# SchlomoFeng/GDN

Measured on AMD Instinct MI355X. Metric: sliding-windows/sec forward+anomaly-score, SWaT-shape (127 sensors, W=15), higher is better.
Workload: dtype f32; 1 GPU; BASELINE configs[2]: SWaT-shape eval forward + anomaly score; sensors=127, window=15, topk=30, dim=64, out_layer_num=1, batch=512, batches_per_launch=64, windows_per_launch=32768, storage=fp32, multi_gpu_measured=False, hip_graph=True, forward_streams=3, parallelism=single GPU

## Files before the change

gdn_amd/csrc/gdn_forward_dense.hip:

```cpp
#include "gdn_common.hpp"

#include <stdlib.h>

int gdn_dense_fused_op_d128(int op, const void* args, int bf16, unsigned* plan_out, long long* bytes,
                            hipStream_t st);

namespace {

typedef _Float16 h8 __attribute__((ext_vector_type(8)));
typedef _Float16 h2 __attribute__((ext_vector_type(2)));
typedef __bf16 b8 __attribute__((ext_vector_type(8)));
typedef __bf16 b2 __attribute__((ext_vector_type(2)));
typedef float f32x16 __attribute__((ext_vector_type(16)));
typedef unsigned int u32x4 __attribute__((ext_vector_type(4)));

enum { FMT_F16 = 0, FMT_BF16 = 1 };
#define GDN_LOG2E 1.44269504088896340736f
#define GDN_F16_ALPHA_SCALE 4096.0f
#define GDN_F16_X_SCALE 8.0f
#define GDN_F16_XT_SCALE 8.0f
#define GDN_F16_Z_SCALE 8.0f

template <int FMT>
struct Fmt;
// ... 48 lines not shown
    for (int j = 0; j < 4; ++j) {
      const unsigned p = Fmt<FMT>::pk(r[2 * j], r[2 * j + 1]);
      out[t][j] = p;
      if (t + 1 < NTERM) {
        r[2 * j] = Fmt<FMT>::res0(p, r[2 * j]);
        r[2 * j + 1] = Fmt<FMT>::res1(p, r[2 * j + 1]);
      }
    }
}

__host__ __device__ __forceinline__ int pos_of_source(int src) {
  return (src & ~12) | ((src & 4) << 1) | ((src & 8) >> 1);
}

enum { DMODE_FUSED = 0 };

template <int NT, int DC, int WK, int SL, int FMT>
struct DCfg {
  static constexpr int KS = 2 * NT;
  static constexpr int ROWS = 32 * NT;
  static constexpr int THREADS = 64 * NT;
  static constexpr int AROW = KS * 32 + 16;
  static constexpr int AWAVE = 32 * AROW;
  static constexpr bool XAGG = FMT == FMT_F16;
  static constexpr int MCB = XAGG ? 1 : DC;
  static constexpr int NPX = FMT == FMT_F16 ? 2 : 1;
  static constexpr int NTL = FMT == FMT_F16 ? 2 : 3;
  static constexpr int NTXIN = FMT == FMT_F16 ? 2 : 1;
  static constexpr int XP = 16 * WK + 4;
  static constexpr int XU = 8 * WK;
  static constexpr bool XHALF = XAGG && WK == 1;
  static constexpr int XFL = XHALF ? 16 : 32;
  static constexpr int XFRAG = 2 * XFL * 16;
  static constexpr int OFF_A = 0;
  static constexpr int OFF_XF = NT * AWAVE;
  static constexpr int OFF_XS = OFF_XF + KS * MCB * NPX * XFRAG;
  static constexpr int OFF_SI = OFF_XS + (XAGG ? 0 : ROWS * XP * 4);
  static constexpr int OFF_SJ = OFF_SI + ROWS * 4;
  static constexpr int OFF_EC = OFF_SJ + ROWS * 4;
  static constexpr int OFF_CS = OFF_EC + 4 * 32 * DC * 4;
  static constexpr int CS_WORDS = XAGG ? 0 : 3 * ROWS;
  static constexpr int LDS = OFF_CS + CS_WORDS * 4;
  static constexpr int CW = 16 * WK, RS = THREADS / CW;
  static __host__ __device__ constexpr int xrow0(int xsl) { return XAGG ? 16 * (xsl >> 1) + 4 * (xsl & 1) : xsl; }
  static __host__ __device__ constexpr int xro(int u) {
    return XAGG ? 16 * NT * (u >> 3) + 8 * ((u & 7) >> 2) + (u & 3) : u * RS;
  }
  static constexpr int LDS_UNIT = 1280;
  static constexpr int LDS_ALLOC = (LDS + LDS_UNIT - 1) / LDS_UNIT * LDS_UNIT;
  static constexpr int WGS = !(DC == 2 && NT >= 3 && SL <= 16 && WK == 1) ? 1
                             : XAGG && 3 * LDS_ALLOC <= 160 * 1024 ? 3 : 2;
};

struct DArgs {
  const void* x;
  int series_len;
  int series_first;
  int batch, n, w, pitch, d;
  const float* lin_w;
  const float* node_terms;
  const uint16_t* nbr;
  const float* gnn_bias;
  const float* emb;
  const float* bn1;
  const float* bn2;
  const float* out_w;
  const float* out_b;
  float* out;
  const unsigned* plan;
  const float* key_gt;
  double* keys;
  int key_pitch;
  int* range_flag;
};

__device__ __forceinline__ float lds_f32(const char* smem, int byte_off) {
  return *reinterpret_cast<const float*>(smem + byte_off);
}
__device__ __forceinline__ u32x4 lds_frag(const char* smem, int byte_off) {
  return *reinterpret_cast<const u32x4*>(smem + byte_off);
}

template <int SL, int FMT, bool WANT_ALPHA>
__device__ __forceinline__ void softmax_split(const char* smem, int si_off, const int (&sjoff)[SL],
                                              unsigned (&ph)[SL / 2], unsigned (&pl)[SL / 2], float (&alpha)[SL]) {
  using F = Fmt<FMT>;
  const float sti = lds_f32(smem, si_off);
  float e[SL];
#pragma unroll
  for (int q = 0; q < SL; ++q) e[q] = lds_f32(smem, sjoff[q]);
  __builtin_amdgcn_sched_barrier(0);
  float m = -3.0e38f;
#pragma unroll
  for (int q = 0; q < SL; ++q) {
    e[q] = leaky(sti + e[q]);
    m = fmaxf(m, e[q]);
  }
  m = fmaxf(m, dpp_f<GDN_DPP_XOR1>(m));
  float sum = 0.f;
#pragma unroll
  for (int q = 0; q < SL; ++q) {
    e[q] = __builtin_amdgcn_exp2f(e[q] - m);
    sum += e[q];
  }
  sum += dpp_f<GDN_DPP_XOR1>(sum);
  constexpr float ASC = FMT == FMT_F16 ? GDN_F16_ALPHA_SCALE : 1.f;
  const float inv = __builtin_amdgcn_rcpf(fmaf(sum, 1.f / ASC, GDN_SOFTMAX_EPS / ASC));
#pragma unroll
  for (int q = 0; q < SL; q += 2) {
    const float a0 = e[q] * inv, a1 = e[q + 1] * inv;
    ph[q / 2] = F::pk(a0, a1);
    pl[q / 2] = F::pk(F::res0(ph[q / 2], a0), F::res1(ph[q / 2], a1));
    if constexpr (WANT_ALPHA) {
      alpha[q] = a0 * (1.f / ASC);
      alpha[q + 1] = a1 * (1.f / ASC);
    }
  }
}

template <int SL>
__device__ __forceinline__ void scatter_terms(char* smem, const int (&scoff)[SL], const unsigned (&p)[SL / 2]) {
#pragma unroll
  for (int q = 0; q < SL; q += 2) {
    *reinterpret_cast<uint16_t*>(smem + scoff[q]) = (uint16_t)p[q / 2];
    *reinterpret_cast<uint16_t*>(smem + scoff[q + 1]) = (uint16_t)(p[q / 2] >> 16);
  }
}

template <int M, int CTRL, int N>
__device__ __forceinline__ void halve_sources(float (&r)[N], bool upper) {
  static_assert(2 * M <= N, "");
#pragma unroll
  for (int i = 0; i < M; ++i) {
    const float keep = upper ? r[i + M] : r[i], give = upper ? r[i] : r[i + M];
    r[i] = keep + dpp_f<CTRL>(give);
  }
}

#ifdef GDN_STAMPS
__device__ unsigned long long g_dense_stamps[64];
#define GDN_STAMP(i)                                                                      \
  if (blockIdx.x == 0 && threadIdx.x == 0) {                                              \
    unsigned long long t_;                                                                \
    asm volatile("s_memrealtime %0\n\ts_waitcnt lgkmcnt(0)" : "=s"(t_)::"memory");       \
    g_dense_stamps[i] = t_;                                                               \
  }
#else
#define GDN_STAMP(i)
#endif

__device__ __forceinline__ float ld_or(const float* p, int idx, bool ok, float other = 0.f) {
  const float v = p[ok ? idx : 0];
  return ok ? v : other;
}

template <int NT, int DC, int WK, int SL, int FMT>
struct LaneConsts {
  using C = DCfg<NT, DC, WK, SL, FMT>;
  int sjoff[SL], scoff[SL];
  u32x4 bl[DC][WK][C::NTL], bs[WK][C::NTL];
  float sk, sp, sadd;
  float e2[DC][16];
  float out_b;
  static constexpr int WORDS = 2 * SL + 4 * DC * WK * C::NTL + (C::XAGG ? 3 : 4 * WK * C::NTL) + 16 * DC + 1;
  static constexpr int TABLE_WORDS = 4 * 32 * DC + C::CS_WORDS;
  static constexpr size_t LIMIT_WORD = (size_t)TABLE_WORDS + (size_t)WORDS * C::THREADS;
  static constexpr size_t PLAN_BYTES = (LIMIT_WORD + 1) * 4;

  template <class Fn>
  __device__ __forceinline__ void each_word(Fn&& f) {
    int i = 0;
#pragma unroll
    for (int q = 0; q < SL; ++q) f(i++, reinterpret_cast<unsigned&>(sjoff[q]));
#pragma unroll
    for (int q = 0; q < SL; ++q) f(i++, reinterpret_cast<unsigned&>(scoff[q]));
#pragma unroll
    for (int cb = 0; cb < DC; ++cb)
#pragma unroll
      for (int wk = 0; wk < WK; ++wk)
#pragma unroll
        for (int t = 0; t < C::NTL; ++t)
#pragma unroll
          for (int e = 0; e < 4; ++e) {
            unsigned tmp = bl[cb][wk][t][e];
            f(i++, tmp);
            bl[cb][wk][t][e] = tmp;
          }
    if constexpr (C::XAGG) {
      f(i++, reinterpret_cast<unsigned&>(sk));
      f(i++, reinterpret_cast<unsigned&>(sp));
      f(i++, reinterpret_cast<unsigned&>(sadd));
    } else {
#pragma unroll
      for (int wk = 0; wk < WK; ++wk)
#pragma unroll
        for (int t = 0; t < C::NTL; ++t)
#pragma unroll
          for (int e = 0; e < 4; ++e) {
            unsigned tmp = bs[wk][t][e];
            f(i++, tmp);
            bs[wk][t][e] = tmp;
          }
    }
#pragma unroll
    for (int cb = 0; cb < DC; ++cb)
#pragma unroll
      for (int r = 0; r < 16; ++r) f(i++, reinterpret_cast<unsigned&>(e2[cb][r]));
    f(i++, reinterpret_cast<unsigned&>(out_b));
  }
};

template <int NT, int DC, int WK, int SL, int FMT>
__device__ __forceinline__ void compute_lane_consts(const DArgs& a, LaneConsts<NT, DC, WK, SL, FMT>& k) {
  using C = DCfg<NT, DC, WK, SL, FMT>;
  constexpr bool FOLD = FMT == FMT_F16;
  const int tid = threadIdx.x, lane = tid & 63, wv = tid >> 6;
  const int l32 = lane & 31, h = lane >> 5;
  const int n = a.n, w = a.w, d = 32 * DC;
  const int ti = 32 * wv + (lane >> 1);
  const int half = lane & 1;
  {
    const uint16_t* row = a.nbr + (size_t)min(ti, n - 1) * a.pitch + half * SL;
#pragma unroll
    for (int q = 0; q < SL; ++q) {
      const int jj = (int)row[q];
      const int j = ti < n ? jj : n;
      k.sjoff[q] = C::OFF_SJ + j * 4;
      k.scoff[q] = C::OFF_A + wv * C::AWAVE + (lane >> 1) * C::AROW + pos_of_source(j) * 2;
    }
  }
#pragma unroll
  for (int cb = 0; cb < DC; ++cb) {
    const int c = cb * 32 + l32;
    const float sc = FOLD ? a.bn1[c] * GDN_F16_X_SCALE : 1.f;
#pragma unroll
    for (int wk = 0; wk < WK; ++wk) {
      float v[8];
#pragma unroll
      for (int j = 0; j < 8; ++j) {
        const int kk = wk * 16 + (C::XAGG ? 8 * (j >> 2) + 4 * h + (j & 3) : 8 * h + j);
        v[j] = ld_or(a.lin_w, c * w + kk, kk < w) * sc;
      }
      split8<FMT, C::NTL>(v, k.bl[cb][wk]);
    }
  }
  if constexpr (C::XAGG) {
    const int xcol = tid & (C::CW - 1), kind = xcol / (C::CW / 2);
    const int pcol = WK == 1 ? xcol ^ 15 : xcol ^ 16;
    const int row = C::xrow0(tid / C::CW) + C::xro(xcol & (C::CW / 2 - 1));
    k.sk = ld_or(a.node_terms, kind * GDN_A_PITCH + xcol, xcol < w) * GDN_LOG2E;
    k.sp = ld_or(a.node_terms, kind * GDN_A_PITCH + pcol, pcol < w) * GDN_LOG2E;
    k.sadd = ld_or(a.node_terms, 2 * GDN_A_PITCH + kind * n + row, row < n) * GDN_LOG2E;
    if (kind == 1 && row == n) k.sadd = -INFINITY;
  } else {
#pragma unroll
    for (int wk = 0; wk < WK; ++wk) {
      float v[8];
#pragma unroll
      for (int j = 0; j < 8; ++j) {
        const int kk = wk * 16 + 8 * h + j;
        v[j] = ld_or(a.node_terms, l32 * GDN_A_PITCH + kk, l32 < 2) * GDN_LOG2E;
      }
      split8<FMT, C::NTL>(v, k.bs[wk]);
    }
  }
  const int tgt = 32 * wv + l32;
#pragma unroll
  for (int cb = 0; cb < DC; ++cb)
#pragma unroll
    for (int r = 0; r < 16; ++r) {
      const int c = cb * 32 + (r & 3) + 8 * (r >> 2) + 4 * h;
      k.e2[cb][r] = ld_or(a.emb, tgt * d + c, tgt < n) * a.bn2[c] *
                    (FMT == FMT_F16 ? 1.f / (GDN_F16_Z_SCALE * GDN_F16_X_SCALE) : 1.f);
    }
  k.out_b = a.out_b[0];
}

template <int NT, int DC, int FMT>
__device__ __forceinline__ void compute_tables(const DArgs& a, float* dst) {
  constexpr int ROWS = 32 * NT, THREADS = 64 * NT, d = 32 * DC;
  const int tid = threadIdx.x, n = a.n;
  for (int c = tid; c < d; c += THREADS) {
    dst[c] = a.bn2[d + c];
    dst[d + c] = a.out_w[c];
    dst[2 * d + c] = a.bn1[c];
    dst[3 * d + c] = fmaf(a.gnn_bias[c], a.bn1[c], a.bn1[d + c]) *
                     (FMT == FMT_F16 ? GDN_F16_Z_SCALE * GDN_F16_X_SCALE : 1.f);
  }
  if constexpr (FMT == FMT_F16) return;
  float* ct = dst + 4 * d;
  for (int t = tid; t < 3 * ROWS; t += THREADS) {
    const int which = t / ROWS, row = t - which * ROWS;
    float v = ld_or(a.node_terms, 2 * GDN_A_PITCH + which * n + row, which < 2 && row < n) * GDN_LOG2E;
    if (which == 1 && row == n) v = -INFINITY;
    ct[t] = v;
  }
}

template <int NT, int DC, int FMT>
__device__ __forceinline__ float compute_xlimit(const DArgs& a) {
  if constexpr (FMT != FMT_F16) return INFINITY;
  __shared__ unsigned m_lin, m_c;
  const int tid = threadIdx.x, d = 32 * DC;
  if (tid == 0) { m_lin = 0u; m_c = 0u; }
  __syncthreads();
  for (int c = tid; c < d; c += 64 * NT) {
    const float sc = a.bn1[c] * GDN_F16_X_SCALE;
    float lmax = 0.f;
    for (int q = 0; q < a.w; ++q) {
      const float v = fabsf(a.lin_w[c * a.w + q] * sc);
      lmax = v > lmax || v != v ? v : lmax;
    }
    const float cin = fabsf(fmaf(a.gnn_bias[c], a.bn1[c], a.bn1[d + c]));
    atomicMax(&m_lin, __float_as_uint(lmax));
    atomicMax(&m_c, __float_as_uint(cin));
  }
  __syncthreads();
  const float lmax = __uint_as_float(m_lin), cmax = __uint_as_float(m_c);
  if (!(lmax < 60000.f) || !(cmax < 3.0e38f)) return 0.f;
  return 60000.f / GDN_F16_XT_SCALE;
}

// ... 91 lines not shown
  }
}
#endif

#ifdef GDN_DENSE_EXTRA_DC
#define GDN_FUSED_ATTR __attribute__((amdgpu_waves_per_eu(1, 1)))
#else
#define GDN_FUSED_ATTR
#endif
#ifndef GDN_K8_PRIO_T
#define GDN_K8_PRIO_T 2
#define GDN_K8_PRIO_S 0
#define GDN_K8_PRIO_M 3
#define GDN_K8_PRIO_Z 1
#endif
#ifndef GDN_PRIO_P
#define GDN_PRIO_P 2
#define GDN_PRIO_S 0
#define GDN_PRIO_M 3
#define GDN_PRIO_E 1
#endif
#ifndef GDN_PRIO_P1
#define GDN_PRIO_P1 3
#endif
template <int NT, int DC, int WK, int SL, int FMT>
__global__ __launch_bounds__(64 * NT, (DCfg<NT, DC, WK, SL, FMT>::WGS)) GDN_FUSED_ATTR void gdn_dense_fused_kernel(const DArgs a) {
  using C = DCfg<NT, DC, WK, SL, FMT>;
  using F = Fmt<FMT>;
  extern __shared__ uint4 smem_u4[];
  char* smem = reinterpret_cast<char*>(smem_u4);
  const int tid = threadIdx.x, lane = tid & 63, wv = tid >> 6;
  const int l32 = lane & 31, h = lane >> 5;
  const int n = a.n, w = a.w, d = 32 * DC;
  constexpr bool FOLD = FMT == FMT_F16;
  GDN_STAMP(0)

  for (int t = lane; t < C::AWAVE / 16; t += 64)
    reinterpret_cast<uint4*>(smem + C::OFF_A + wv * C::AWAVE)[t] = make_uint4(0, 0, 0, 0);
  {
  }
  LaneConsts<NT, DC, WK, SL, FMT> k;
  float xlim = INFINITY;
  if (a.plan) {
    const unsigned* lanes = a.plan + LaneConsts<NT, DC, WK, SL, FMT>::TABLE_WORDS;
    k.each_word([&](int i, unsigned& wd) { wd = lanes[i * C::THREADS + tid]; });
    unsigned* tab = reinterpret_cast<unsigned*>(smem + C::OFF_EC);
    for (int t = tid; t < LaneConsts<NT, DC, WK, SL, FMT>::TABLE_WORDS; t += C::THREADS) tab[t] = a.plan[t];
    if constexpr (FMT == FMT_F16)
      if (a.range_flag) xlim = __uint_as_float(a.plan[LaneConsts<NT, DC, WK, SL, FMT>::LIMIT_WORD]);
  } else {
    compute_lane_consts(a, k);
    compute_tables<NT, DC, FMT>(a, reinterpret_cast<float*>(smem + C::OFF_EC));
  }
  unsigned long long out_of_range = 0ull;
  const int si_off = C::OFF_SI + (32 * wv + (lane >> 1)) * 4;
  const int cs_off = C::OFF_CS + (min(l32, 2) * C::ROWS + 32 * wv + 4 * h) * 4;
  const int tgt = 32 * wv + l32;

  constexpr int CW = C::CW, RS = C::RS;
  static_assert(C::XU * RS == C::ROWS, "x staging covers the tile");
  static_assert(!C::XAGG || RS * WK == 2 * C::KS, "one operand slot per thread and pass");
  constexpr int ESZ = FMT == FMT_F16 ? 4 : 2;
  const int xcol = tid & (CW - 1), xsl = tid / CW;
  const int xrow0 = C::xrow0(xsl);
  auto xro = [](int u) constexpr { return C::xro(u); };
  const int rstride = a.series_len > 0 ? a.series_len : w;
  const int xvoff = (min(xrow0, n - 1) * rstride + min(xcol, w - 1)) * ESZ;
  const int xstep = rstride * ESZ;
  const int xst_off = C::OFF_XS + (xrow0 * C::XP + xcol) * 4;
  const int xf_st = C::OFF_XF + (xsl >> 1) * C::NPX * C::XFRAG + ((xsl & 1) * C::XFL + xcol) * 16;
  const int xs_dst = (xcol / (CW / 2) ? C::OFF_SJ : C::OFF_SI) + (xrow0 + C::xro(xcol & (CW / 2 - 1))) * 4;
  bool xok[C::XU];
#pragma unroll
  for (int u = 0; u < C::XU; ++u) xok[u] = xcol < w && xrow0 + xro(u) < n;
  const size_t win_stride = a.series_len > 0 ? 1 : (size_t)n * w;
  const size_t x0 = a.series_len > 0 ? (size_t)a.series_first : 0;
  const size_t x_total = (a.series_len > 0 ? (size_t)n * a.series_len : (size_t)a.batch * n * w) * ESZ;
  float xr[C::XU];
  auto load_window = [&](int bb) {
    const size_t first = (x0 + (size_t)bb * win_stride) * ESZ;
    const size_t rem = x_total - first;
    const __amdgpu_buffer_rsrc_t rsrc = __builtin_amdgcn_make_buffer_rsrc(
        const_cast<char*>(reinterpret_cast<const char*>(a.x)) + first, 0,
        (int)(rem > 0xffffffffull ? 0xffffffffu : (unsigned)rem), 0x00020000);
#pragma unroll
    for (int u = 0; u < C::XU; ++u) {
      if constexpr (FMT == FMT_F16) {
        xr[u] = __uint_as_float(__builtin_amdgcn_raw_buffer_load_b32(rsrc, xvoff, xro(u) * xstep, 0));
      } else {
        xr[u] = __uint_as_float((unsigned)__builtin_amdgcn_raw_buffer_load_b16(rsrc, xvoff, xro(u) * xstep, 0) << 16);
      }
    }
  };
  GDN_STAMP(1)
  load_window(blockIdx.x);
  __syncthreads();
  GDN_STAMP(2)

  const int arow_off = C::OFF_A + wv * C::AWAVE + l32 * C::AROW + h * 16;
  const int xrow_off = C::OFF_XS + ((32 * wv + l32) * C::XP + 8 * h) * 4;
  const int ec_off = C::OFF_EC + 16 * h;

  for (int b = blockIdx.x; b < a.batch; b += gridDim.x) {
    if constexpr (C::XAGG) {
      __builtin_amdgcn_s_setprio(GDN_PRIO_P);
      if (b == (int)blockIdx.x) { GDN_STAMP(3) }
      __syncthreads();
      float xv[C::XU];
#pragma unroll
      for (int u = 0; u < C::XU; ++u) {
        xv[u] = xok[u] ? xr[u] : 0.f;
#ifndef GDN_NO_GUARD
        out_of_range |= __builtin_amdgcn_ballot_w64(!(fabsf(xv[u]) < xlim));
#endif
      }
#pragma unroll
      for (int q = 0; q < WK; ++q) {
        float v[8];
#pragma unroll
        for (int j = 0; j < 8; ++j) v[j] = xv[8 * q + j] * GDN_F16_XT_SCALE;
        u32x4 xf[C::NPX];
        split8<FMT, C::NPX>(v, xf);
#pragma unroll
        for (int t = 0; t < C::NPX; ++t)
          *reinterpret_cast<u32x4*>(smem + xf_st + (q * NT * C::NPX + t) * C::XFRAG) = xf[t];
      }
      float sr[C::XU];
#pragma unroll
      for (int u = 0; u < C::XU; ++u) {
        const float other = WK == 1 ? dpp_f<GDN_DPP_MIRROR>(xv[u]) : __shfl_xor(xv[u], 16);
        sr[u] = fmaf(other, k.sp, xv[u] * k.sk);
      }
      if constexpr (WK == 2) halve_sources<8, GDN_DPP_MIRROR>(sr, (xcol & 8) != 0);
      halve_sources<4, GDN_DPP_HALF_MIRROR>(sr, (xcol & 4) != 0);
      halve_sources<2, GDN_DPP_XOR3>(sr, (xcol & 2) != 0);
      halve_sources<1, GDN_DPP_XOR1>(sr, (xcol & 1) != 0);
      *reinterpret_cast<float*>(smem + xs_dst) = sr[0] + k.sadd;
      load_window(min(b + (int)gridDim.x, a.batch - 1));
      if (b == (int)blockIdx.x) { GDN_STAMP(4) }
    } else {
#pragma unroll
      for (int u = 0; u < C::XU; ++u) {
        const float xv = xok[u] ? xr[u] : 0.f;
        *reinterpret_cast<float*>(smem + xst_off + xro(u) * (C::XP * 4)) = xv;
      }
      if (b == (int)blockIdx.x) { GDN_STAMP(3) }
      __syncthreads();
      load_window(min(b + (int)gridDim.x, a.batch - 1));
      if (b == (int)blockIdx.x) { GDN_STAMP(4) }

      {
        __builtin_amdgcn_s_setprio(GDN_PRIO_P);
        f32x16 acc1[DC], accs;
#pragma unroll
        for (int cb = 0; cb < DC; ++cb)
#pragma unroll
          for (int r = 0; r < 16; ++r) acc1[cb][r] = 0.f;
#pragma unroll
        for (int g = 0; g < 4; ++g) {
          const float4 t = *reinterpret_cast<const float4*>(smem + cs_off + 32 * g);
          accs[4 * g] = t.x; accs[4 * g + 1] = t.y; accs[4 * g + 2] = t.z; accs[4 * g + 3] = t.w;
        }
#pragma unroll
        for (int wk = 0; wk < WK; ++wk) {
          float v[8];
          const float4 v0 = *reinterpret_cast<const float4*>(smem + xrow_off + wk * 64);
          const float4 v1 = *reinterpret_cast<const float4*>(smem + xrow_off + wk * 64 + 16);
          v[0] = v0.x; v[1] = v0.y; v[2] = v0.z; v[3] = v0.w;
          v[4] = v1.x; v[5] = v1.y; v[6] = v1.z; v[7] = v1.w;
          u32x4 ax[C::NTXIN];
// ... 6 lines not shown
#pragma unroll
                for (int cb = 0; cb < DC; ++cb) acc1[cb] = F::mfma(ax[tx], k.bl[cb][wk][tl], acc1[cb]);
                accs = F::mfma(ax[tx], k.bs[wk][tl], accs);
              }
        }
        if (l32 < 2) {
          float* sdst = reinterpret_cast<float*>(smem + (l32 == 0 ? C::OFF_SI : C::OFF_SJ)) + 32 * wv + 4 * h;
#pragma unroll
          for (int r = 0; r < 16; ++r) sdst[(r & 3) + 8 * (r >> 2)] = accs[r];
        }
#pragma unroll
        for (int cb = 0; cb < DC; ++cb)
#pragma unroll
          for (int s = 0; s < 2; ++s) {
            float v[8];
#pragma unroll
            for (int j = 0; j < 8; ++j) v[j] = acc1[cb][8 * s + j];
            u32x4 xf[C::NPX];
            split8<FMT, C::NPX>(v, xf);
#pragma unroll
            for (int t = 0; t < C::NPX; ++t)
              *reinterpret_cast<u32x4*>(smem + C::OFF_XF + ((((2 * wv + s) * DC + cb) * C::NPX + t) << 10) + lane * 16) = xf[t];
          }
      }
    }
    __builtin_amdgcn_s_setprio(GDN_PRIO_S);
    if (b == (int)blockIdx.x) { GDN_STAMP(5) }
    __syncthreads();
    if (b == (int)blockIdx.x) { GDN_STAMP(6) }

    unsigned ph[SL / 2], pl[SL / 2];
    {
      float unused[SL];
      softmax_split<SL, FMT, false>(smem, si_off, k.sjoff, ph, pl, unused);
    }
    float ygt = 0.f;
    if (a.keys && h == 0 && tgt < n) ygt = a.key_gt[(size_t)b * n + tgt];
    constexpr int MCB = C::MCB;
    f32x16 acc2[MCB];
#pragma unroll
    for (int cb = 0; cb < MCB; ++cb)
#pragma unroll
      for (int r = 0; r < 16; ++r) acc2[cb][r] = 0.f;
    constexpr int XF_KS = MCB * C::NPX * C::XFRAG;
    const int xf_lane = C::OFF_XF + (C::XHALF ? h * 16 + (l32 & 15) : lane) * 16;
    u32x4 fa[2], fx[2][MCB][C::NPX];
    auto fetch_hi = [&](int ks, int buf) {
      fa[buf] = lds_frag(smem, arow_off + ks * 32);
#pragma unroll
      for (int cb = 0; cb < MCB; ++cb)
#pragma unroll
        for (int t = 0; t < C::NPX; ++t) fx[buf][cb][t] = lds_frag(smem, xf_lane + ks * XF_KS + (cb * C::NPX + t) * C::XFRAG);
    };
    auto fetch_lo = [&](int ks, int buf) {
      fa[buf] = lds_frag(smem, arow_off + ks * 32);
#pragma unroll
      for (int cb = 0; cb < MCB; ++cb) fx[buf][cb][0] = lds_frag(smem, xf_lane + ks * XF_KS + cb * C::NPX * C::XFRAG);
    };
    if (b == (int)blockIdx.x) { GDN_STAMP(7) }
    __builtin_amdgcn_s_setprio(GDN_PRIO_M);
    scatter_terms<SL>(smem, k.scoff, ph);
    __builtin_amdgcn_sched_barrier(0);
    fetch_hi(0, 0);
    __builtin_amdgcn_sched_barrier(0);
#pragma unroll
    for (int ks = 0; ks < C::KS; ++ks) {
      if (ks + 1 < C::KS) fetch_hi(ks + 1, (ks + 1) & 1);
      __builtin_amdgcn_sched_barrier(0);
#pragma unroll
      for (int cb = 0; cb < MCB; ++cb)
#pragma unroll
        for (int t = 0; t < C::NPX; ++t) acc2[cb] = F::mfma(fx[ks & 1][cb][t], fa[ks & 1], acc2[cb]);
      __builtin_amdgcn_sched_barrier(0);
    }
    scatter_terms<SL>(smem, k.scoff, pl);
    __builtin_amdgcn_sched_barrier(0);
    fetch_lo(0, 0);
    __builtin_amdgcn_sched_barrier(0);
#pragma unroll
    for (int ks = 0; ks < C::KS; ++ks) {
      if (ks + 1 < C::KS) fetch_lo(ks + 1, (ks + 1) & 1);
      __builtin_amdgcn_sched_barrier(0);
#pragma unroll
      for (int cb = 0; cb < MCB; ++cb) acc2[cb] = F::mfma(fx[ks & 1][cb][0], fa[ks & 1], acc2[cb]);
      __builtin_amdgcn_sched_barrier(0);
    }
    if (b == (int)blockIdx.x) { GDN_STAMP(8) }
    f32x16 acc3[DC];
    if constexpr (C::XAGG) {
      __builtin_amdgcn_s_setprio(GDN_PRIO_P1);
#pragma unroll
      for (int cb = 0; cb < DC; ++cb)
#pragma unroll
        for (int g = 0; g < 4; ++g) {
          const float4 t = *reinterpret_cast<const float4*>(smem + ec_off + 12 * d + 128 * cb + 32 * g);
          acc3[cb][4 * g] = t.x; acc3[cb][4 * g + 1] = t.y; acc3[cb][4 * g + 2] = t.z; acc3[cb][4 * g + 3] = t.w;
        }
#pragma unroll
      for (int wk = 0; wk < WK; ++wk) {
        float v[8];
#pragma unroll
        for (int j = 0; j < 8; ++j)
          v[j] = acc2[0][8 * wk + j] * (GDN_F16_Z_SCALE / (GDN_F16_ALPHA_SCALE * GDN_F16_XT_SCALE));
        u32x4 zf[2];
        split8<FMT, 2>(v, zf);
#pragma unroll
        for (int tz = 0; tz < 2; ++tz)
#pragma unroll
          for (int tl = 0; tl < C::NTL; ++tl)
            if (tz + tl < 2) {
#pragma unroll
              for (int cb = 0; cb < DC; ++cb) acc3[cb] = F::mfma(k.bl[cb][wk][tl], zf[tz], acc3[cb]);
            }
      }
    } else {
#pragma unroll
      for (int cb = 0; cb < DC; ++cb) acc3[cb] = acc2[cb < MCB ? cb : 0];
    }

    __builtin_amdgcn_s_setprio(GDN_PRIO_E);
    if (b == (int)blockIdx.x) { GDN_STAMP(9) }
    float part = 0.f;
#pragma unroll
    for (int cb = 0; cb < DC; ++cb)
#pragma unroll
      for (int g = 0; g < 4; ++g) {
        const float4 sh2 = *reinterpret_cast<const float4*>(smem + ec_off + 128 * cb + 32 * g);
        const float4 wo = *reinterpret_cast<const float4*>(smem + ec_off + 4 * d + 128 * cb + 32 * g);
        const float sh2a[4] = {sh2.x, sh2.y, sh2.z, sh2.w}, woa[4] = {wo.x, wo.y, wo.z, wo.w};
        float sc1a[4] = {1.f, 1.f, 1.f, 1.f}, sh1a[4] = {0.f, 0.f, 0.f, 0.f};
        if constexpr (!FOLD) {
          const float4 t0 = *reinterpret_cast<const float4*>(smem + ec_off + 8 * d + 128 * cb + 32 * g);
          const float4 t1 = *reinterpret_cast<const float4*>(smem + ec_off + 12 * d + 128 * cb + 32 * g);
          sc1a[0] = t0.x; sc1a[1] = t0.y; sc1a[2] = t0.z; sc1a[3] = t0.w;
          sh1a[0] = t1.x; sh1a[1] = t1.y; sh1a[2] = t1.z; sh1a[3] = t1.w;
        }
#pragma unroll
        for (int i = 0; i < 4; ++i) {
          float v = acc3[cb][4 * g + i];
          if constexpr (!FOLD) v = fmaf(v, sc1a[i], sh1a[i]);
          v = fmaxf(v, 0.f);
          v = fmaxf(fmaf(v, k.e2[cb][4 * g + i], sh2a[i]), 0.f);
          part = fmaf(v, woa[i], part);
        }
      }
    part += __shfl_xor(part, 32);
    if (h == 0 && tgt < n) {
      const float o = part + k.out_b;
      a.out[(size_t)b * n + tgt] = o;
      if (a.keys) a.keys[(size_t)tgt * a.key_pitch + b] = fabs((double)o - (double)ygt);
    }
    if (b == (int)blockIdx.x) { GDN_STAMP(10) }
  }
  if constexpr (FMT == FMT_F16)
    if (a.range_flag && out_of_range != 0ull && lane == 0) a.range_flag[0] = 1;
  GDN_STAMP(11)
}

#ifndef GDN_DENSE_EXTRA_DC
typedef short s16x4 __attribute__((ext_vector_type(4)));

template <int NT, int SL, int FMT>
struct KCfg {
  static constexpr int KS = 2 * NT;
  static constexpr int ROWS = 32 * NT;
  static constexpr int THREADS = 64 * NT;
  static constexpr int AROW = KS * 32 + 16;
  static constexpr int AWAVE = 32 * AROW;
  static constexpr int NPX = FMT == FMT_F16 ? 2 : 1;
  static constexpr int TPLANE = ROWS * 128;
  static constexpr int OFF_A = 0;
  static constexpr int OFF_T = NT * AWAVE;
  static constexpr int OFF_SI = OFF_T + NPX * TPLANE;
  static constexpr int OFF_SJ = OFF_SI + ROWS * 4;
  static constexpr int LDS = OFF_SJ + ROWS * 4;
  static constexpr int PPR = FMT == FMT_F16 ? 16 : 8;
  static constexpr int RSTEP = THREADS / PPR;
  static constexpr int TU = ROWS / RSTEP;
};

struct KArgs {
  const void* xlin;
  const float* si;
  const float* sj;
  const uint16_t* nbr;
// ... 651 lines not shown
            for (int cb = 0; cb < DC; ++cb) acc1[cb] = F::mfma(ax[tx], bl[cb][wk][tl], acc1[cb]);
            accs = F::mfma(ax[tx], bs[wk][tl], accs);
          }
    }
    __syncthreads();
#pragma unroll
    for (int r = 0; r < 16; ++r) {
      const int row = 32 * wv + (r & 3) + 8 * (r >> 2) + 4 * h;
      if (row < n) {
        const size_t grow = (size_t)b * n + row;
        if (l32 == 0) a.si[grow] = accs[r];
        if (l32 == 1) a.sj[grow] = accs[r];
      }
#pragma unroll
      for (int cb = 0; cb < DC; ++cb) {
        const float v = acc1[cb][r];
        if constexpr (FMT == FMT_F16) {
          if (row < n) reinterpret_cast<float*>(a.xlin)[((size_t)b * n + row) * 64 + cb * 32 + l32] = v;
        } else {
          const float nb = dpp_f<GDN_DPP_XOR1>(v);
          if (row < n && (lane & 1) == 0)
            reinterpret_cast<unsigned*>(a.xlin)[(((size_t)b * n + row) * 64 + cb * 32 + l32) >> 1] = F::pk(v, nb);
        }
      }
    }
  }
}

#endif

static inline int blocks_per_cu(const void* fn, int threads, int lds) { return gdn_blocks_per_cu(fn, threads, lds); }
static inline int cu_count() { return gdn_cu_count(); }

enum { DOP_LAUNCH = 0, DOP_PLAN_BUILD = 1, DOP_PLAN_BYTES = 2 };

template <int NT, int DC, int WK, int SL, int FMT>
int fused_op(int op, const DArgs& a, unsigned* plan_out, long long* bytes, hipStream_t stream) {
  using C = DCfg<NT, DC, WK, SL, FMT>;
  using K = LaneConsts<NT, DC, WK, SL, FMT>;
  static_assert(C::LDS <= 160 * 1024, "LDS plan exceeds one CU");
  static_assert(C::OFF_CS == C::OFF_EC + 4 * 32 * DC * 4, "the two LDS tables are one block of the plan");
  if (op == DOP_PLAN_BYTES) {
    *bytes = (long long)K::PLAN_BYTES;
    return GDN_OK;
  }
  if (op == DOP_PLAN_BUILD) {
    hipLaunchKernelGGL((gdn_dense_plan_kernel<NT, DC, WK, SL, FMT>), dim3(1), dim3(C::THREADS), 0, stream, a, plan_out);
    return gdn_launch_status();
  }
  auto kern = gdn_dense_fused_kernel<NT, DC, WK, SL, FMT>;
  const int occ = blocks_per_cu(reinterpret_cast<const void*>(kern), C::THREADS, C::LDS);
  if (occ < C::WGS) return GDN_ERR_LAUNCH;
  const int occ_cap = GDN_ENV_INT_ONCE("GDN_DENSE_MAX_OCC", 0);
  const int occ_used = occ_cap > 0 ? min(occ, occ_cap) : occ;
  const int slots = cu_count() * occ_used;
  int wpw = GDN_ENV_INT_ONCE("GDN_DENSE_MIN_WPW", 0);
  if (wpw <= 0) wpw = (a.batch > cu_count() && a.batch <= slots) ? 2 : 1;
  const int grid = max(1, min((a.batch + wpw - 1) / wpw, slots));
  hipLaunchKernelGGL(kern, dim3(grid), dim3(C::THREADS), C::LDS, stream, a);
  return gdn_launch_status();
}

template <int NT, int DC, int WK, int FMT>
int select_sl(int op, const DArgs& a, unsigned* plan_out, long long* bytes, hipStream_t st) {
  switch (a.pitch) {
    case 16: return fused_op<NT, DC, WK, 8, FMT>(op, a, plan_out, bytes, st);
    case 32: return fused_op<NT, DC, WK, 16, FMT>(op, a, plan_out, bytes, st);
    case 48: return fused_op<NT, DC, WK, 24, FMT>(op, a, plan_out, bytes, st);
    case 64: return fused_op<NT, DC, WK, 32, FMT>(op, a, plan_out, bytes, st);
  }
  return GDN_ERR_UNSUPPORTED;
}

template <int NT, int FMT, int DC>
int select_wk(int op, const DArgs& a, unsigned* plan_out, long long* bytes, hipStream_t st) {
  if (a.w <= 16) return select_sl<NT, DC, 1, FMT>(op, a, plan_out, bytes, st);
  return select_sl<NT, DC, 2, FMT>(op, a, plan_out, bytes, st);
}

template <int FMT, int DC>
int select_nt(int op, const DArgs& a, unsigned* plan_out, long long* bytes, hipStream_t st) {
  switch ((a.n + 1 + 31) / 32) {
    case 1: return select_wk<1, FMT, DC>(op, a, plan_out, bytes, st);
    case 2: return select_wk<2, FMT, DC>(op, a, plan_out, bytes, st);
// ... 110 lines not shown
                             hipStream_t stream) {
  if (!gdn_dense_supported(n, 1, d, k)) return GDN_ERR_UNSUPPORTED;
  KArgs a = {};
  a.xlin = xlin; a.si = s_i; a.sj = s_j; a.nbr = nbr; a.bias = bias;
  a.batch = batch; a.n = n; a.pitch = gdn_nbr_pitch(k); a.z = z; a.alpha = alpha;
  if (is_bf16) return alpha ? attn_select_nt<FMT_BF16, true>(a, stream) : attn_select_nt<FMT_BF16, false>(a, stream);
  return alpha ? attn_select_nt<FMT_F16, true>(a, stream) : attn_select_nt<FMT_F16, false>(a, stream);
}

bool gdn_dense_supported(int n, int w, int d, int k) {
  return n >= 1 && n <= 127 && d == 64 && w >= 1 && w <= 32 && k >= 1 && k <= n && gdn_nbr_pitch(k) <= 64;
}
bool gdn_dense_fused_supported(int n, int w, int d, int k) {
  return gdn_dense_supported(n, w, 64, k) && (d == 64 || d == 128);
}

static int fused_dispatch(int op, const DArgs& a, int bf16, unsigned* plan_out, long long* bytes, hipStream_t st) {
  if (a.d == 128) return gdn_dense_fused_op_d128(op, &a, bf16, plan_out, bytes, st);
  return bf16 ? select_nt<FMT_BF16, 2>(op, a, plan_out, bytes, st) : select_nt<FMT_F16, 2>(op, a, plan_out, bytes, st);
}

int gdn_dense_forward_fused(const void* x, int x_is_bf16, int series_len, int series_first, const float* lin_w,
                            const float* node_terms, const uint16_t* nbr, const float* gnn_bias,
                            const float* emb, const float* bn1, const float* bn2, const float* out_w,
                            const float* out_b, int batch, int n, int w, int d, int k, float* out,
                            hipStream_t stream) {
  if (!gdn_dense_fused_supported(n, w, d, k)) return GDN_ERR_UNSUPPORTED;
  DArgs a = {};
  a.x = x; a.series_len = series_len; a.series_first = series_first;
  a.batch = batch; a.n = n; a.w = w; a.pitch = gdn_nbr_pitch(k); a.d = d;
  a.lin_w = lin_w; a.node_terms = node_terms; a.nbr = nbr; a.gnn_bias = gnn_bias; a.emb = emb;
  a.bn1 = bn1; a.bn2 = bn2; a.out_w = out_w; a.out_b = out_b; a.out = out;
  return fused_dispatch(DOP_LAUNCH, a, x_is_bf16, nullptr, nullptr, stream);
}

#ifdef GDN_STAMPS
extern "C" int gdn_debug_read_stamps(unsigned long long* host_out) {
  return hipMemcpyFromSymbol(host_out, HIP_SYMBOL(g_dense_stamps), sizeof(g_dense_stamps)) == hipSuccess ? 0 : -2;
}
#endif

template <int NT>
static int bank_order_select_sl(const uint16_t* nbr, int n, int pitch, uint16_t* out, hipStream_t st) {
  switch (pitch) {
    case 16: hipLaunchKernelGGL((gdn_bank_order_kernel<NT, 8>), dim3(1), dim3(64 * NT), 0, st, nbr, n, pitch, out); break;
    case 32: hipLaunchKernelGGL((gdn_bank_order_kernel<NT, 16>), dim3(1), dim3(64 * NT), 0, st, nbr, n, pitch, out); break;
    case 48: hipLaunchKernelGGL((gdn_bank_order_kernel<NT, 24>), dim3(1), dim3(64 * NT), 0, st, nbr, n, pitch, out); break;
    case 64: hipLaunchKernelGGL((gdn_bank_order_kernel<NT, 32>), dim3(1), dim3(64 * NT), 0, st, nbr, n, pitch, out); break;
    default: return GDN_ERR_UNSUPPORTED;
  }
  return gdn_launch_status();
}

extern "C" int gdn_graph_bank_order(const uint16_t* nbr, int n, int k, uint16_t* nbr_ordered, void* stream) {
  if (!nbr || !nbr_ordered || n <= 0 || k <= 0) return GDN_ERR_ARG;
  if (!gdn_dense_supported(n, 1, 64, k)) return GDN_ERR_UNSUPPORTED;
  const int pitch = gdn_nbr_pitch(k);
  hipStream_t st = (hipStream_t)stream;
  switch ((n + 1 + 31) / 32) {
    case 1: return bank_order_select_sl<1>(nbr, n, pitch, nbr_ordered, st);
    case 2: return bank_order_select_sl<2>(nbr, n, pitch, nbr_ordered, st);
    case 3: return bank_order_select_sl<3>(nbr, n, pitch, nbr_ordered, st);
    case 4: return bank_order_select_sl<4>(nbr, n, pitch, nbr_ordered, st);
  }
  return GDN_ERR_UNSUPPORTED;
}
// ... 77 lines not shown
```

Baseline: 142.0 million windows/s.

## Transpose f16 output MFMA so channels map to lanes and reduce via permlane

For the f16 aggregated path, the output MFMA operands are swapped so the accumulator holds targets along rows and channels along lanes. Per-channel constants (bias shift, bn2 shift, out_w) become per-lane scalars in registers instead of float4 LDS reads, and the final dot product is reduced across lanes with permlane16 swap and DPP steps. The LDS epilogue table shrinks to two rows for this path, and stores are issued by even lanes with remapped targets. This trades the per-element LDS table loads for a cross-lane reduction and more lane-constant registers.

```diff
diff --git a/gdn_amd/csrc/gdn_forward_dense.hip b/gdn_amd/csrc/gdn_forward_dense.hip
--- a/gdn_amd/csrc/gdn_forward_dense.hip
+++ b/gdn_amd/csrc/gdn_forward_dense.hip
@@ -110,7 +110,8 @@
   static constexpr int OFF_SI = OFF_XS + (XAGG ? 0 : ROWS * XP * 4);
   static constexpr int OFF_SJ = OFF_SI + ROWS * 4;
   static constexpr int OFF_EC = OFF_SJ + ROWS * 4;
-  static constexpr int OFF_CS = OFF_EC + 4 * 32 * DC * 4;
+  static constexpr int EC_WORDS = (XAGG ? 2 : 4) * 32 * DC;
+  static constexpr int OFF_CS = OFF_EC + EC_WORDS * 4;
   static constexpr int CS_WORDS = XAGG ? 0 : 3 * ROWS;
   static constexpr int LDS = OFF_CS + CS_WORDS * 4;
   static constexpr int CW = 16 * WK, RS = THREADS / CW;
@@ -209,6 +210,18 @@
   }
 }
 
+__device__ __forceinline__ float column_sum_to_lanes(float (&p)[16], int l32) {
+#pragma unroll
+  for (int i = 0; i < 8; ++i) {
+    const auto s = __builtin_amdgcn_permlane16_swap(__float_as_uint(p[i]), __float_as_uint(p[i + 8]), false, false);
+    p[i] = __uint_as_float(s[0]) + __uint_as_float(s[1]);
+  }
+  halve_sources<4, GDN_DPP_MIRROR>(p, (l32 & 8) != 0);
+  halve_sources<2, GDN_DPP_HALF_MIRROR>(p, (l32 & 4) != 0);
+  halve_sources<1, GDN_DPP_XOR3>(p, (l32 & 2) != 0);
+  return p[0] + dpp_f<GDN_DPP_XOR1>(p[0]);
+}
+
 #ifdef GDN_STAMPS
 __device__ unsigned long long g_dense_stamps[64];
 #define GDN_STAMP(i)                                                                      \
@@ -232,10 +245,12 @@
   int sjoff[SL], scoff[SL];
   u32x4 bl[DC][WK][C::NTL], bs[WK][C::NTL];
   float sk, sp, sadd;
+  float wo[DC];
   float e2[DC][16];
   float out_b;
-  static constexpr int WORDS = 2 * SL + 4 * DC * WK * C::NTL + (C::XAGG ? 3 : 4 * WK * C::NTL) + 16 * DC + 1;
-  static constexpr int TABLE_WORDS = 4 * 32 * DC + C::CS_WORDS;
+  static constexpr int WORDS =
+      2 * SL + 4 * DC * WK * C::NTL + (C::XAGG ? 3 + DC : 4 * WK * C::NTL) + 16 * DC + 1;
+  static constexpr int TABLE_WORDS = C::EC_WORDS + C::CS_WORDS;
   static constexpr size_t LIMIT_WORD = (size_t)TABLE_WORDS + (size_t)WORDS * C::THREADS;
   static constexpr size_t PLAN_BYTES = (LIMIT_WORD + 1) * 4;
 
@@ -262,6 +277,8 @@
       f(i++, reinterpret_cast<unsigned&>(sk));
       f(i++, reinterpret_cast<unsigned&>(sp));
       f(i++, reinterpret_cast<unsigned&>(sadd));
+#pragma unroll
+      for (int cb = 0; cb < DC; ++cb) f(i++, reinterpret_cast<unsigned&>(wo[cb]));
     } else {
 #pragma unroll
       for (int wk = 0; wk < WK; ++wk)
@@ -324,6 +341,8 @@
     k.sp = ld_or(a.node_terms, kind * GDN_A_PITCH + pcol, pcol < w) * GDN_LOG2E;
     k.sadd = ld_or(a.node_terms, 2 * GDN_A_PITCH + kind * n + row, row < n) * GDN_LOG2E;
     if (kind == 1 && row == n) k.sadd = -INFINITY;
+#pragma unroll
+    for (int cb = 0; cb < DC; ++cb) k.wo[cb] = a.out_w[cb * 32 + l32];
   } else {
 #pragma unroll
     for (int wk = 0; wk < WK; ++wk) {
@@ -336,12 +355,12 @@
       split8<FMT, C::NTL>(v, k.bs[wk]);
     }
   }
-  const int tgt = 32 * wv + l32;
 #pragma unroll
   for (int cb = 0; cb < DC; ++cb)
 #pragma unroll
     for (int r = 0; r < 16; ++r) {
-      const int c = cb * 32 + (r & 3) + 8 * (r >> 2) + 4 * h;
+      const int row = (r & 3) + 8 * (r >> 2) + 4 * h;
+      const int tgt = 32 * wv + (C::XAGG ? row : l32), c = cb * 32 + (C::XAGG ? l32 : row);
       k.e2[cb][r] = ld_or(a.emb, tgt * d + c, tgt < n) * a.bn2[c] *
                     (FMT == FMT_F16 ? 1.f / (GDN_F16_Z_SCALE * GDN_F16_X_SCALE) : 1.f);
     }
@@ -352,14 +371,19 @@
 __device__ __forceinline__ void compute_tables(const DArgs& a, float* dst) {
   constexpr int ROWS = 32 * NT, THREADS = 64 * NT, d = 32 * DC;
   const int tid = threadIdx.x, n = a.n;
+  if constexpr (FMT == FMT_F16) {
+    for (int c = tid; c < d; c += THREADS) {
+      dst[c] = fmaf(a.gnn_bias[c], a.bn1[c], a.bn1[d + c]) * (GDN_F16_Z_SCALE * GDN_F16_X_SCALE);
+      dst[d + c] = a.bn2[d + c];
+    }
+    return;
+  }
   for (int c = tid; c < d; c += THREADS) {
     dst[c] = a.bn2[d + c];
     dst[d + c] = a.out_w[c];
     dst[2 * d + c] = a.bn1[c];
-    dst[3 * d + c] = fmaf(a.gnn_bias[c], a.bn1[c], a.bn1[d + c]) *
-                     (FMT == FMT_F16 ? GDN_F16_Z_SCALE * GDN_F16_X_SCALE : 1.f);
-  }
-  if constexpr (FMT == FMT_F16) return;
+    dst[3 * d + c] = fmaf(a.gnn_bias[c], a.bn1[c], a.bn1[d + c]);
+  }
   float* ct = dst + 4 * d;
   for (int t = tid; t < 3 * ROWS; t += THREADS) {
     const int which = t / ROWS, row = t - which * ROWS;
@@ -517,7 +541,6 @@
   const int tid = threadIdx.x, lane = tid & 63, wv = tid >> 6;
   const int l32 = lane & 31, h = lane >> 5;
   const int n = a.n, w = a.w, d = 32 * DC;
-  constexpr bool FOLD = FMT == FMT_F16;
   GDN_STAMP(0)
 
   for (int t = lane; t < C::AWAVE / 16; t += 64)
@@ -540,7 +563,8 @@
   unsigned long long out_of_range = 0ull;
   const int si_off = C::OFF_SI + (32 * wv + (lane >> 1)) * 4;
   const int cs_off = C::OFF_CS + (min(l32, 2) * C::ROWS + 32 * wv + 4 * h) * 4;
-  const int tgt = 32 * wv + l32;
+  const int tgt = C::XAGG ? 32 * wv + 8 * (l32 >> 3) + 4 * h + ((l32 >> 1) & 3) : 32 * wv + l32;
+  const bool stores = (C::XAGG ? (lane & 1) == 0 : h == 0) && tgt < n;
 
   constexpr int CW = C::CW, RS = C::RS;
   static_assert(C::XU * RS == C::ROWS, "x staging covers the tile");
@@ -584,7 +608,7 @@
 
   const int arow_off = C::OFF_A + wv * C::AWAVE + l32 * C::AROW + h * 16;
   const int xrow_off = C::OFF_XS + ((32 * wv + l32) * C::XP + 8 * h) * 4;
-  const int ec_off = C::OFF_EC + 16 * h;
+  const int ec_off = C::OFF_EC + (C::XAGG ? 4 * l32 : 16 * h);
 
   for (int b = blockIdx.x; b < a.batch; b += gridDim.x) {
     if constexpr (C::XAGG) {
@@ -696,7 +720,7 @@
       softmax_split<SL, FMT, false>(smem, si_off, k.sjoff, ph, pl, unused);
     }
     float ygt = 0.f;
-    if (a.keys && h == 0 && tgt < n) ygt = a.key_gt[(size_t)b * n + tgt];
+    if (a.keys && stores) ygt = a.key_gt[(size_t)b * n + tgt];
     constexpr int MCB = C::MCB;
     f32x16 acc2[MCB];
 #pragma unroll
@@ -751,12 +775,11 @@
     if constexpr (C::XAGG) {
       __builtin_amdgcn_s_setprio(GDN_PRIO_P1);
 #pragma unroll
-      for (int cb = 0; cb < DC; ++cb)
-#pragma unroll
-        for (int g = 0; g < 4; ++g) {
-          const float4 t = *reinterpret_cast<const float4*>(smem + ec_off + 12 * d + 128 * cb + 32 * g);
-          acc3[cb][4 * g] = t.x; acc3[cb][4 * g + 1] = t.y; acc3[cb][4 * g + 2] = t.z; acc3[cb][4 * g + 3] = t.w;
-        }
+      for (int cb = 0; cb < DC; ++cb) {
+        const float cin = lds_f32(smem, ec_off + 128 * cb);
+#pragma unroll
+        for (int r = 0; r < 16; ++r) acc3[cb][r] = cin;
+      }
 #pragma unroll
       for (int wk = 0; wk < WK; ++wk) {
         float v[8];
@@ -771,7 +794,7 @@
           for (int tl = 0; tl < C::NTL; ++tl)
             if (tz + tl < 2) {
 #pragma unroll
-              for (int cb = 0; cb < DC; ++cb) acc3[cb] = F::mfma(k.bl[cb][wk][tl], zf[tz], acc3[cb]);
+              for (int cb = 0; cb < DC; ++cb) acc3[cb] = F::mfma(zf[tz], k.bl[cb][wk][tl], acc3[cb]);
             }
       }
     } else {
@@ -782,31 +805,41 @@
     __builtin_amdgcn_s_setprio(GDN_PRIO_E);
     if (b == (int)blockIdx.x) { GDN_STAMP(9) }
     float part = 0.f;
-#pragma unroll
-    for (int cb = 0; cb < DC; ++cb)
-#pragma unroll
-      for (int g = 0; g < 4; ++g) {
-        const float4 sh2 = *reinterpret_cast<const float4*>(smem + ec_off + 128 * cb + 32 * g);
-        const float4 wo = *reinterpret_cast<const float4*>(smem + ec_off + 4 * d + 128 * cb + 32 * g);
-        const float sh2a[4] = {sh2.x, sh2.y, sh2.z, sh2.w}, woa[4] = {wo.x, wo.y, wo.z, wo.w};
-        float sc1a[4] = {1.f, 1.f, 1.f, 1.f}, sh1a[4] = {0.f, 0.f, 0.f, 0.f};
-        if constexpr (!FOLD) {
-          const float4 t0 = *reinterpret_cast<const float4*>(smem + ec_off + 8 * d + 128 * cb + 32 * g);
-          const float4 t1 = *reinterpret_cast<const float4*>(smem + ec_off + 12 * d + 128 * cb + 32 * g);
-          sc1a[0] = t0.x; sc1a[1] = t0.y; sc1a[2] = t0.z; sc1a[3] = t0.w;
-          sh1a[0] = t1.x; sh1a[1] = t1.y; sh1a[2] = t1.z; sh1a[3] = t1.w;
+    if constexpr (C::XAGG) {
+      float p[16], sh2[DC];
+#pragma unroll
+      for (int cb = 0; cb < DC; ++cb) sh2[cb] = lds_f32(smem, ec_off + 128 * (DC + cb));
+#pragma unroll
+      for (int r = 0; r < 16; ++r) {
+#pragma unroll
+        for (int cb = 0; cb < DC; ++cb) {
+          float v = fmaxf(acc3[cb][r], 0.f);
+          v = fmaxf(fmaf(v, k.e2[cb][r], sh2[cb]), 0.f);
+          p[r] = cb == 0 ? v * k.wo[0] : fmaf(v, k.wo[cb], p[r]);
         }
-#pragma unroll
-        for (int i = 0; i < 4; ++i) {
-          float v = acc3[cb][4 * g + i];
-          if constexpr (!FOLD) v = fmaf(v, sc1a[i], sh1a[i]);
-          v = fmaxf(v, 0.f);
-          v = fmaxf(fmaf(v, k.e2[cb][4 * g + i], sh2a[i]), 0.f);
-          part = fmaf(v, woa[i], part);
+      }
+      part = column_sum_to_lanes(p, l32);
+    } else {
+#pragma unroll
+      for (int cb = 0; cb < DC; ++cb)
+#pragma unroll
+        for (int g = 0; g < 4; ++g) {
+          const float4 sh2 = *reinterpret_cast<const float4*>(smem + ec_off + 128 * cb + 32 * g);
+          const float4 wo = *reinterpret_cast<const float4*>(smem + ec_off + 4 * d + 128 * cb + 32 * g);
+          const float4 sc1 = *reinterpret_cast<const float4*>(smem + ec_off + 8 * d + 128 * cb + 32 * g);
+          const float4 sh1 = *reinterpret_cast<const float4*>(smem + ec_off + 12 * d + 128 * cb + 32 * g);
+          const float sh2a[4] = {sh2.x, sh2.y, sh2.z, sh2.w}, woa[4] = {wo.x, wo.y, wo.z, wo.w};
+          const float sc1a[4] = {sc1.x, sc1.y, sc1.z, sc1.w}, sh1a[4] = {sh1.x, sh1.y, sh1.z, sh1.w};
+#pragma unroll
+          for (int i = 0; i < 4; ++i) {
+            float v = fmaxf(fmaf(acc3[cb][4 * g + i], sc1a[i], sh1a[i]), 0.f);
+            v = fmaxf(fmaf(v, k.e2[cb][4 * g + i], sh2a[i]), 0.f);
+            part = fmaf(v, woa[i], part);
+          }
         }
-      }
-    part += __shfl_xor(part, 32);
-    if (h == 0 && tgt < n) {
+      part += __shfl_xor(part, 32);
+    }
+    if (stores) {
       const float o = part + k.out_b;
       a.out[(size_t)b * n + tgt] = o;
       if (a.keys) a.keys[(size_t)tgt * a.key_pitch + b] = fabs((double)o - (double)ygt);
@@ -1536,7 +1569,7 @@
   using C = DCfg<NT, DC, WK, SL, FMT>;
   using K = LaneConsts<NT, DC, WK, SL, FMT>;
   static_assert(C::LDS <= 160 * 1024, "LDS plan exceeds one CU");
-  static_assert(C::OFF_CS == C::OFF_EC + 4 * 32 * DC * 4, "the two LDS tables are one block of the plan");
+  static_assert(C::OFF_CS == C::OFF_EC + C::EC_WORDS * 4, "the two LDS tables are one block of the plan");
   if (op == DOP_PLAN_BYTES) {
     *bytes = (long long)K::PLAN_BYTES;
     return GDN_OK;
```

After: 139.1 million windows/s. 0.98x the previous value.

## Double-buffer LDS x-fragments and s_j to drop per-iteration barrier

Applied to the files above, without the earlier changes.

For the f16 XAGG three-workgroup shape, the x-fragment and s_j LDS regions are double-buffered and alternate each batch iteration, so the barrier at the top of the loop can be skipped. This removes one workgroup-wide sync per window batch and lets waves overlap staging of the next batch with consumption of the current one. It costs extra LDS, guarded by a static_assert that three workgroups still fit per CU. It also adds an occupancy query entry point for debugging.

```diff
diff --git a/gdn_amd/csrc/gdn_forward_dense.hip b/gdn_amd/csrc/gdn_forward_dense.hip
--- a/gdn_amd/csrc/gdn_forward_dense.hip
+++ b/gdn_amd/csrc/gdn_forward_dense.hip
@@ -104,12 +104,17 @@
   static constexpr bool XHALF = XAGG && WK == 1;
   static constexpr int XFL = XHALF ? 16 : 32;
   static constexpr int XFRAG = 2 * XFL * 16;
+  static constexpr bool W3SHAPE = DC == 2 && NT >= 3 && SL <= 16 && WK == 1;
+  static constexpr bool ONEBAR = XAGG && W3SHAPE;
+  static constexpr int NBUF = ONEBAR ? 2 : 1;
+  static constexpr int XF_BYTES = KS * MCB * NPX * XFRAG;
+  static constexpr int SJ_BYTES = ROWS * 4;
   static constexpr int OFF_A = 0;
   static constexpr int OFF_XF = NT * AWAVE;
-  static constexpr int OFF_XS = OFF_XF + KS * MCB * NPX * XFRAG;
+  static constexpr int OFF_XS = OFF_XF + NBUF * XF_BYTES;
   static constexpr int OFF_SI = OFF_XS + (XAGG ? 0 : ROWS * XP * 4);
   static constexpr int OFF_SJ = OFF_SI + ROWS * 4;
-  static constexpr int OFF_EC = OFF_SJ + ROWS * 4;
+  static constexpr int OFF_EC = OFF_SJ + NBUF * SJ_BYTES;
   static constexpr int OFF_CS = OFF_EC + 4 * 32 * DC * 4;
   static constexpr int CS_WORDS = XAGG ? 0 : 3 * ROWS;
   static constexpr int LDS = OFF_CS + CS_WORDS * 4;
@@ -120,8 +125,9 @@
   }
   static constexpr int LDS_UNIT = 1280;
   static constexpr int LDS_ALLOC = (LDS + LDS_UNIT - 1) / LDS_UNIT * LDS_UNIT;
-  static constexpr int WGS = !(DC == 2 && NT >= 3 && SL <= 16 && WK == 1) ? 1
-                             : XAGG && 3 * LDS_ALLOC <= 160 * 1024 ? 3 : 2;
+  static constexpr int WGS = !W3SHAPE ? 1 : XAGG && 3 * LDS_ALLOC <= 160 * 1024 ? 3 : 2;
+  static_assert(!ONEBAR || WGS == 3, "the double-buffered LDS map must leave room for three workgroups per CU");
+  static_assert(OFF_SJ % 128 == 0 && SJ_BYTES % 128 == 0, "the plan's bank order of the s_j gather assumes it");
 };
 
 struct DArgs {
@@ -155,12 +161,13 @@
 
 template <int SL, int FMT, bool WANT_ALPHA>
 __device__ __forceinline__ void softmax_split(const char* smem, int si_off, const int (&sjoff)[SL],
-                                              unsigned (&ph)[SL / 2], unsigned (&pl)[SL / 2], float (&alpha)[SL]) {
+                                              unsigned (&ph)[SL / 2], unsigned (&pl)[SL / 2], float (&alpha)[SL],
+                                              int sj_par = 0) {
   using F = Fmt<FMT>;
   const float sti = lds_f32(smem, si_off);
   float e[SL];
 #pragma unroll
-  for (int q = 0; q < SL; ++q) e[q] = lds_f32(smem, sjoff[q]);
+  for (int q = 0; q < SL; ++q) e[q] = lds_f32(smem, sjoff[q] + sj_par);
   __builtin_amdgcn_sched_barrier(0);
   float m = -3.0e38f;
 #pragma unroll
@@ -586,11 +593,13 @@
   const int xrow_off = C::OFF_XS + ((32 * wv + l32) * C::XP + 8 * h) * 4;
   const int ec_off = C::OFF_EC + 16 * h;
 
+  int pxf = 0, psj = 0;
   for (int b = blockIdx.x; b < a.batch; b += gridDim.x) {
     if constexpr (C::XAGG) {
       __builtin_amdgcn_s_setprio(GDN_PRIO_P);
       if (b == (int)blockIdx.x) { GDN_STAMP(3) }
-      __syncthreads();
+      if constexpr (!C::ONEBAR)
+        __syncthreads();
       float xv[C::XU];
 #pragma unroll
       for (int u = 0; u < C::XU; ++u) {
@@ -608,7 +617,7 @@
         split8<FMT, C::NPX>(v, xf);
 #pragma unroll
         for (int t = 0; t < C::NPX; ++t)
-          *reinterpret_cast<u32x4*>(smem + xf_st + (q * NT * C::NPX + t) * C::XFRAG) = xf[t];
+          *reinterpret_cast<u32x4*>(smem + xf_st + pxf + (q * NT * C::NPX + t) * C::XFRAG) = xf[t];
       }
       float sr[C::XU];
 #pragma unroll
@@ -620,7 +629,7 @@
       halve_sources<4, GDN_DPP_HALF_MIRROR>(sr, (xcol & 4) != 0);
       halve_sources<2, GDN_DPP_XOR3>(sr, (xcol & 2) != 0);
       halve_sources<1, GDN_DPP_XOR1>(sr, (xcol & 1) != 0);
-      *reinterpret_cast<float*>(smem + xs_dst) = sr[0] + k.sadd;
+      *reinterpret_cast<float*>(smem + xs_dst + (xcol / (CW / 2)) * psj) = sr[0] + k.sadd;
       load_window(min(b + (int)gridDim.x, a.batch - 1));
       if (b == (int)blockIdx.x) { GDN_STAMP(4) }
     } else {
@@ -693,7 +702,7 @@
     unsigned ph[SL / 2], pl[SL / 2];
     {
       float unused[SL];
-      softmax_split<SL, FMT, false>(smem, si_off, k.sjoff, ph, pl, unused);
+      softmax_split<SL, FMT, false>(smem, si_off, k.sjoff, ph, pl, unused, psj);
     }
     float ygt = 0.f;
     if (a.keys && h == 0 && tgt < n) ygt = a.key_gt[(size_t)b * n + tgt];
@@ -704,7 +713,7 @@
 #pragma unroll
       for (int r = 0; r < 16; ++r) acc2[cb][r] = 0.f;
     constexpr int XF_KS = MCB * C::NPX * C::XFRAG;
-    const int xf_lane = C::OFF_XF + (C::XHALF ? h * 16 + (l32 & 15) : lane) * 16;
+    const int xf_lane = C::OFF_XF + pxf + (C::XHALF ? h * 16 + (l32 & 15) : lane) * 16;
     u32x4 fa[2], fx[2][MCB][C::NPX];
     auto fetch_hi = [&](int ks, int buf) {
       fa[buf] = lds_frag(smem, arow_off + ks * 32);
@@ -812,6 +821,10 @@
       if (a.keys) a.keys[(size_t)tgt * a.key_pitch + b] = fabs((double)o - (double)ygt);
     }
     if (b == (int)blockIdx.x) { GDN_STAMP(10) }
+    if constexpr (C::ONEBAR) {
+      pxf ^= C::XF_BYTES;
+      psj ^= C::SJ_BYTES;
+    }
   }
   if constexpr (FMT == FMT_F16)
     if (a.range_flag && out_of_range != 0ull && lane == 0) a.range_flag[0] = 1;
@@ -1529,7 +1542,7 @@
 static inline int blocks_per_cu(const void* fn, int threads, int lds) { return gdn_blocks_per_cu(fn, threads, lds); }
 static inline int cu_count() { return gdn_cu_count(); }
 
-enum { DOP_LAUNCH = 0, DOP_PLAN_BUILD = 1, DOP_PLAN_BYTES = 2 };
+enum { DOP_LAUNCH = 0, DOP_PLAN_BUILD = 1, DOP_PLAN_BYTES = 2, DOP_OCCUPANCY = 3 };
 
 template <int NT, int DC, int WK, int SL, int FMT>
 int fused_op(int op, const DArgs& a, unsigned* plan_out, long long* bytes, hipStream_t stream) {
@@ -1547,6 +1560,10 @@
   }
   auto kern = gdn_dense_fused_kernel<NT, DC, WK, SL, FMT>;
   const int occ = blocks_per_cu(reinterpret_cast<const void*>(kern), C::THREADS, C::LDS);
+  if (op == DOP_OCCUPANCY) {
+    *bytes = occ;
+    return GDN_OK;
+  }
   if (occ < C::WGS) return GDN_ERR_LAUNCH;
   const int occ_cap = GDN_ENV_INT_ONCE("GDN_DENSE_MAX_OCC", 0);
   const int occ_used = occ_cap > 0 ? min(occ, occ_cap) : occ;
@@ -1723,6 +1740,15 @@
   a.lin_w = lin_w; a.node_terms = node_terms; a.nbr = nbr; a.gnn_bias = gnn_bias; a.emb = emb;
   a.bn1 = bn1; a.bn2 = bn2; a.out_w = out_w; a.out_b = out_b; a.out = out;
   return fused_dispatch(DOP_LAUNCH, a, x_is_bf16, nullptr, nullptr, stream);
+}
+
+extern "C" int gdn_debug_fused_blocks_per_cu(int n, int w, int d, int k, int bf16_storage) {
+  if (!gdn_dense_fused_supported(n, w, d, k)) return 0;
+  DArgs a = {};
+  a.n = n; a.w = w; a.d = d; a.pitch = gdn_nbr_pitch(k);
+  long long occ = 0;
+  const int rc = fused_dispatch(DOP_OCCUPANCY, a, bf16_storage, nullptr, &occ, nullptr);
+  return rc == GDN_OK ? (int)occ : 0;
 }
 
 #ifdef GDN_STAMPS
```

Result: slower. 142.5 million windows/s before, 140.9 million windows/s after (-1.1%).
